# qpc001/Feature_Base_Pointcloud_Registration

Measured on AMD Instinct MI355X. Metric: registered scans/sec + pose RMSE vs ref, 64×1800 synthetic Velodyne, higher is better.
Workload: dtype f32; 1 GPU; C2: 64x1800 HDL-64-style scans, ~100k-pt local corner+surf map; 1024 independent scan-to-map jobs per GPU per step (C4-style independent jobs); parallelism=single GPU, imu_deskew=False, exact_voxel_order=0

## Files before the change

feature_base_pointcloud_registration_amd/csrc/fbr_api.hip:

```cpp
#include <hip/hip_runtime.h>

#include <algorithm>
#include <atomic>
#include <chrono>
#include <condition_variable>
#include <cmath>
#include <cstdio>
#include <cstdlib>
#include <cstring>
#include <dlfcn.h>
#include <functional>
#include <map>
#include <mutex>
#include <set>
#include <string>
#include <thread>
#include <vector>

#include "fbr_common.h"
#include "fbr_imu.h"
#include "fbr_kernels.h"
#include "fbr_msg.h"

using namespace fbr;
// ... 443 lines not shown
  if (!sb.stream_mode && !pk && !c->staged_24) return FBR_ERR_STATE;
  int32_t* owner = c->d_owner + j0 * c->HW;
  OwnerTag ot;
  const int trc = next_owner_tag(c, &ot);
  if (trc) return trc;
  TIMED_ON(c, sb.st, "project", launch_project(sb.st, c->d_pts + i0 * c->NMAX, c->d_nin + i0, c->NMAX, sb.B, c->H,
                                               c->W, owner, c->d_err + j0, sb.stream_mode ? c->single_n : -1, pk, ot));
  TIMED_ON(c, sb.st, "extract",
           launch_extract(sb.st, c->d_pts + i0 * c->NMAX, c->NMAX, owner, sb.B, c->H, c->W, c->d_rowcnt + j0 * c->H,
                          c->d_choff + j0 * c->H * (c->W / 32 + 1),
                          c->d_cloud + j0 * c->HW, c->d_col + j0 * c->HW, c->d_range + j0 * c->HW,
                          c->d_start + j0 * c->H, c->d_end + j0 * c->H, c->d_nvalid + j0, desk, pk, ot));
  return FBR_OK;
}

bool packed_scans_enabled() {
  static const bool v = [] {
    const char* e = std::getenv("FBR_PACKED_SCANS");
    return e ? std::atoi(e) != 0 : true;
  }();
  return v;
}

bool feat_surf_window() {
  static const bool v = [] {
    const char* e = std::getenv("FBR_FEAT_SURF_WINDOW");
    return e ? std::atoi(e) != 0 : true;
  }();
  return v;
}

int stage_features(fbr_ctx* c, const Sub& sb, bool stream_mode, bool err_clear = false, bool labels_out = false) {
  const int64_t j0 = sb.j0, HW = c->HW, H = c->H;
  FeatArgs a{};
  a.B = sb.B;
  a.H = c->H;
  a.W = c->W;
  a.cloud = c->d_cloud + j0 * HW;
  a.col = c->d_col + j0 * HW;
  a.range = c->d_range + j0 * HW;
  a.start_ring = c->d_start + j0 * H;
  a.end_ring = c->d_end + j0 * H;
  a.nvalid = c->d_nvalid + j0;
  a.edge_thr = c->P.edge_threshold;
  a.surf_thr = c->P.surf_threshold;
  if (stream_mode) {
    a.stream = c->d_sstream;
    a.label = c->d_label_stream;
  } else {
    CK(hipMemsetAsync(c->d_sstate + j0, 0, sizeof(StreamState) * sb.B, sb.st));
    a.stream = c->d_sstate + j0;
    a.label = c->d_label + j0 * HW;
  }
  a.corner_slot = c->d_corner_slot + j0 * H * kCornerPerRing;
  a.corner_cnt = c->d_corner_cnt + j0 * H;
  a.err = c->d_err + j0;
  a.surf_full = labels_out || !feat_surf_window() ? 1 : 0;
  a.carry = stream_mode ? 1 : 0;
  a.fresh = stream_mode ? 0 : 1;
  feat_caps(c->W, a);
  a.gscratch = c->d_feat_scratch + j0 * H * a.gslot_bytes;
  a.stamps = c->d_feat_stamps ? c->d_feat_stamps + j0 * H * 12 : nullptr;
  if (!err_clear) CK(hipMemsetAsync(c->d_err + j0, 0, sizeof(int32_t) * sb.B, sb.st));
  TIMED_ON(c, sb.st, "features", launch_features(sb.st, a));
  if (!stream_mode && c->diag_err_job >= sb.in0 && c->diag_err_job < sb.in0 + sb.B)
    CK(hipMemsetD32Async((hipDeviceptr_t)(c->d_err + j0 + (c->diag_err_job - sb.in0)), 1, 1, sb.st));
  VgRing v{};
  v.cloud = a.cloud;
  v.label = a.label;
  v.start_ring = a.start_ring;
  v.end_ring = a.end_ring;
  v.B = sb.B;
  v.H = c->H;
  v.HW = HW;
  v.cap = c->W;
  v.leaf = c->P.odometry_surf_leaf_size;
  v.out = c->d_surf_ring + j0 * HW;
  v.stride_out = c->W;
  v.cnt_out = c->d_surf_ring_cnt + j0 * H;
  v.dbg = std::getenv("FBR_VR_DBG") ? std::atoi(std::getenv("FBR_VR_DBG")) : 0;
  v.exact = c->P.exact_voxel_order ? 1 : 0;
  v.stamps = a.stamps;
  v.kernel = c->diag_ring_filter;
  TIMED_ON(c, sb.st, "voxel_ring", launch_voxel_ring(sb.st, v));
  TIMED_ON(c, sb.st, "concat",
           launch_concat(sb.st, sb.B, c->H, c->W, a.corner_slot, a.corner_cnt, v.out, v.cnt_out,
                         c->d_corner_all + j0 * HW, HW, c->d_ncorner + j0, c->d_surf_all + j0 * HW, HW,
                         c->d_nsurf + j0, c->d_ring_box + j0 * H * kRingBox));
  c->ring_box_valid = true;
  return FBR_OK;
}

GnArgs gn_args(fbr_ctx* c, const Sub& sb, bool trace) {
  const int64_t j0 = sb.j0, HW = c->HW, ib = j0 * c->items_per_job;
  const int mi = std::max(1, c->P.max_iterations);
  GnArgs a{};
#ifdef FBR_KNN_STATS
  a.knn_stats = knn_stats_buffer();
#endif
  a.B = sb.B;
  a.max_iter = c->P.max_iterations;
  a.cornerDS = c->d_cornerDS + j0 * HW;
  a.capc = HW;
  a.ncds = c->d_ncds + j0;
  a.surfDS = c->d_surfDS + j0 * HW;
  a.caps = HW;
  a.nsds = c->d_nsds + j0;
  a.mc = c->grid_c.view();
  a.ms = c->grid_s.view();
  a.gn = c->d_gn + j0;
  a.guess = c->d_guess + (int64_t)sb.in0 * 6;
  a.items = c->d_items + ib;
  a.nitems = c->d_nitems + sb.k;
  a.item_range = c->d_item_range + j0 * 2;
  a.partial = c->d_partial + ib * 32;
  a.max_items = sb.B * c->items_per_job;
  a.edge_min = c->P.edge_feature_min_valid_num;
  a.surf_min = c->P.surf_feature_min_valid_num;
  for (int k = 0; k < 3; ++k) a.crop_half[k] = c->P.crop_half[k];
  a.rot_tol = c->P.rotation_tollerance;
  a.z_tol = c->P.z_tollerance;
  a.pose_out = c->d_pose_out + j0 * 6;
  a.stats = c->d_stats + j0;
  a.trace = trace ? c->d_trace + j0 * c->P.max_iterations * 6 : nullptr;
  a.nbr = c->d_nbr + ib * 5 * 256;
  a.fitc = c->d_fitc + ib * 6 * 256;
  a.fits = c->d_fits + ib * 256;
  a.nsame = c->d_nsame + ib * 256;
  static const int fit_cache = [] {
    const char* e = std::getenv("FBR_FIT_CACHE");
    return e ? std::atoi(e) : 1;
  }();
  a.fit_cache = fit_cache;
  a.iter_flags = c->d_iter_flags + (int64_t)sb.k * mi;
  a.items_flag = c->d_iter_flags + (int64_t)kMaxSub * mi + sb.k;
  a.iter_cnt = c->d_iter_cnt + (int64_t)sb.k * 4 * mi;
  if (c->d_bin) {
    const int64_t slots = (int64_t)c->max_items * 256;
    a.fb_list = c->d_fb_list + ib * 256;
    a.bin_list = c->d_fb_list + slots + ib * 256;
    a.qblk = c->d_fb_list + 2 * slots + ib * 256;
    a.bin = c->d_bin + (int64_t)sb.k * 3 * c->bin_nb;
    a.nb_c = (int)c->bin_nb_c;
    a.nb_s = (int)(c->bin_nb - c->bin_nb_c);
  }
  a.desk_mode = c->desk_any ? c->d_desk_mode + sb.in0 : nullptr;
  a.desk = c->desk_any ? c->d_desk + sb.in0 : nullptr;
  a.nocrop = c->map_nocrop ? 1 : 0;
  a.deg_carry = sb.stream_mode ? c->stream_degenerate : 0;
  if (c->direct_gen && sb.stream_mode && sb.B == 1 && c->d_direct) {
    a.direct = c->d_direct;
    a.direct_done = c->d_direct_done;
    a.direct_gen = c->direct_gen;
    a.nvalid = c->d_nvalid + j0;
    a.ncorner = c->d_ncorner + j0;
    a.nsurf = c->d_nsurf + j0;
    a.ferr = c->d_err + j0;
    a.cropcnt = c->d_cropcnt + (int64_t)sb.in0 * 2;
  }
  return a;
}

int batch_quiesce(fbr_ctx* c);
int drop_staged_batch(fbr_ctx* c) {
  const int rc = batch_quiesce(c);
  c->staged_B = 0;
// ... 1799 lines not shown
}

}

int fbr_process_batch(fbr_ctx* c, const fbr_point_xyzirt* const* scans, const int64_t* n_in, int n_jobs,
                      float* poses_inout, fbr_reg_stats* stats) {
  if (!c || !scans || !n_in || !poses_inout || n_jobs < 0) return FBR_ERR_INVALID_ARG;
  for (int j = 0; j < n_jobs; ++j) {
    if (n_in[j] < 0 || n_in[j] > c->NMAX) return FBR_ERR_CAPACITY;
    if (n_in[j] && !scans[j]) return FBR_ERR_INVALID_ARG;
  }
  if (n_jobs == 0) return FBR_OK;
  if (!c->has_map) return FBR_ERR_NO_MAP;
  CK(enter(c));
  int rc = ingest_init(c);
  if (rc) return rc;
  c->ing.h2d_bytes = 0.0;
  const int nb = (n_jobs + c->Bcap - 1) / c->Bcap;
  auto first = [&](int b) { return b * c->Bcap; };
  auto count = [&](int b) { return std::min(c->Bcap, n_jobs - b * c->Bcap); };
  rc = ingest_upload(c, 0, scans, n_in, count(0));
  for (int b = 0; b < nb && !rc; ++b) {
    const int slot = b & 1, j0 = first(b), B = count(b);
    int up_rc = FBR_OK;
    std::thread up;
    if (b + 1 < nb)
      up = std::thread([&, b] { up_rc = ingest_upload(c, slot ^ 1, scans + first(b + 1), n_in + first(b + 1), count(b + 1)); });
    rc = ingest_stage(c, slot, n_in + j0, B, poses_inout + 6 * j0);
    if (!rc) rc = fbr_batch_launch(c);
    if (!rc) rc = fbr_batch_wait(c);
    if (!rc) rc = fbr_batch_results(c, poses_inout + 6 * j0, stats ? stats + j0 : nullptr);
    if (up.joinable()) up.join();
    if (!rc) rc = up_rc;
  }
  (void)fbr_sync(c->ing.cstream);
  if (c->ing.xstream) (void)fbr_sync(c->ing.xstream);
  c->d_pts = c->ing.d_pts_slot[0];
  if (rc) (void)drop_staged_batch(c);
  return rc;
}

int fbr_debug_counters(long long* launches, long long* host_syncs, long long* flag_polls, int reset) {
  DebugCounters& d = debug_counters();
  if (launches) *launches = d.launches.load();
  if (host_syncs) *host_syncs = d.host_syncs.load();
  if (flag_polls) *flag_polls = d.flag_polls.load();
  if (reset) {
    d.launches = 0;
    d.host_syncs = 0;
    d.flag_polls = 0;
  }
  return FBR_OK;
}

extern "C" int fbr_diag_host_times(long long* out4, int reset) {
  DebugCounters& d = debug_counters();
  for (int k = 0; k < 4; ++k) {
    if (out4) out4[k] = d.host_ns[k].load();
    if (reset) d.host_ns[k] = 0;
  }
  return FBR_OK;
}

extern "C" int fbr_diag_wait_stats(long long* out4, int reset) {
  DebugCounters& d = debug_counters();
  std::atomic<long long>* v[4] = {&d.flag_fallbacks, &d.waits_over_1ms, &d.wait_max_ns, &d.stream_queries};
  for (int k = 0; k < 4; ++k) {
    if (out4) out4[k] = v[k]->load();
    if (reset) *v[k] = 0;
  }
  return FBR_OK;
}

extern "C" int fbr_diag_batch_times(long long* out2, int reset) {
  DebugCounters& d = debug_counters();
  for (int k = 0; k < 2; ++k) {
    if (out2) out2[k] = d.batch_ns[k].load();
    if (reset) d.batch_ns[k] = 0;
  }
  return FBR_OK;
}

extern "C" int fbr_diag_ring_filter(fbr_ctx* c, int kernel) {
  if (!c || (kernel != -1 && kernel != 0 && kernel != 2)) return FBR_ERR_INVALID_ARG;
  c->diag_ring_filter = kernel;
  return FBR_OK;
}

extern "C" int fbr_diag_force_capacity_error(fbr_ctx* c, int job) {
  if (!c) return FBR_ERR_INVALID_ARG;
  c->diag_err_job = job < 0 ? -1 : job;
  return FBR_OK;
}

int fbr_ingest_bytes(fbr_ctx* c, double* h2d_bytes) {
  if (!c || !h2d_bytes) return FBR_ERR_INVALID_ARG;
  *h2d_bytes = c->ing.h2d_bytes;
  return FBR_OK;
}

int fbr_voxel_grid(fbr_ctx* c, const fbr_point_xyzi* in, int64_t n, float leaf, fbr_point_xyzi* out, int64_t* n_out) {
  if (!c || n < 0 || (n && !in) || !(leaf > 0)) return FBR_ERR_INVALID_ARG;
  CK(enter(c));
  std::vector<fbr_point_xyzi> o;
  int rc = voxel_grid_once(c, in, n, leaf, o);
  if (rc) return rc;
  if (out) std::memcpy(out, o.data(), sizeof(fbr_point_xyzi) * o.size());
  if (n_out) *n_out = (int64_t)o.size();
  return FBR_OK;
}

extern "C" int fbr_diag_feature_stamps(fbr_ctx* c, unsigned long long* out ) {
  if (!c) return FBR_ERR_INVALID_ARG;
  CK(enter(c));
  const size_t n = (size_t)c->Bwork * c->H * 12;
  if (!c->d_feat_stamps) {
    CK(hipMalloc(&c->d_feat_stamps, sizeof(unsigned long long) * n));
    CK(hipMemset(c->d_feat_stamps, 0, sizeof(unsigned long long) * n));
    return FBR_OK;
  }
  if (out) CK(fbr_memcpy_sync(out, c->d_feat_stamps, sizeof(unsigned long long) * n, hipMemcpyDeviceToHost));
  return FBR_OK;
}

int fbr_set_profiling(fbr_ctx* c, int enable) {
  if (!c) return FBR_ERR_INVALID_ARG;
  c->profiling = enable != 0;
  return FBR_OK;
}

int fbr_set_profiling_kernels(fbr_ctx* c, const char* names) {
  if (!c) return FBR_ERR_INVALID_ARG;
  c->profile_only.clear();
  if (!names) return FBR_OK;
  std::string cur;
  for (const char* q = names;; ++q) {
    if (*q == ',' || *q == '\0') {
      if (!cur.empty()) c->profile_only.insert(cur);
      cur.clear();
      if (*q == '\0') break;
    } else {
      cur.push_back(*q);
    }
  }
  return FBR_OK;
}

int fbr_kernel_time(fbr_ctx* c, const char* kernel, double* total_ms, int64_t* launches) {
  if (!c || !kernel) return FBR_ERR_INVALID_ARG;
  CK(enter(c));
  auto itr = c->timers.find(kernel);
  if (itr == c->timers.end()) {
    if (total_ms) *total_ms = 0.0;
    if (launches) *launches = 0;
    return FBR_OK;
  }
  KernelTimer& t = itr->second;
  for (auto& pr : t.pending) {
    CK(hipEventSynchronize(pr.second));
    float ms = 0.0f;
    CK(hipEventElapsedTime(&ms, pr.first, pr.second));
    t.total_ms += ms;
    t.launches += 1;
    t.pool.push_back(pr);
  }
  t.pending.clear();
  if (total_ms) *total_ms = t.total_ms;
// ... 203 lines not shown
```

feature_base_pointcloud_registration_amd/csrc/fbr_kernels.h:

```cpp
#pragma once
#include <hip/hip_ext.h>
#include <hip/hip_runtime.h>
#include <stdint.h>

#include <algorithm>
#include <atomic>

#include "fbr_common.h"

namespace fbr {

struct LaunchTimer {
  hipEvent_t start = nullptr, stop = nullptr;
  int launched = 0;
};
inline LaunchTimer& launch_timer() {
  static thread_local LaunchTimer t;
  return t;
}

struct DebugCounters {
  std::atomic<long long> launches{0}, host_syncs{0}, flag_polls{0};
  std::atomic<long long> host_ns[4] = {0, 0, 0, 0};
  std::atomic<long long> batch_ns[2] = {0, 0};
// ... 68 lines not shown
  int surf_full = 1;
  int carry = 0;
  int fresh = 0;
};
size_t features_lds_bytes(const FeatArgs& a, int nwv);
size_t features_gslot_bytes(const FeatArgs& a);
void launch_features(hipStream_t s, const FeatArgs& a);

struct VgSet {
  const float4* in;
  int64_t stride_in;
  const int32_t* cnt_in;
  int64_t cap;
  float4* out;
  int64_t stride_out;
  int32_t* cnt_out;
  uint32_t* scratch;
  float leaf;
  int nseg;
  int morton;
  int exact;
  const float* box;
  int box_n;
  int64_t box_stride;
};
constexpr int64_t kVgScratch = 5;
struct VgArgs {
  VgSet s[2];
  int32_t* err = nullptr;
};
constexpr int32_t kVgErrLookback = 16;
constexpr int64_t kVgLdsCap = 4096;
void launch_voxel_grid(hipStream_t s, const VgArgs& a);

struct DevArena {
  char* base = nullptr;
  size_t cap = 0, used = 0;
};
inline size_t arena_bytes(size_t b) { return (std::max<size_t>(b, 1) + 255) & ~(size_t)255; }
inline hipError_t arena_reserve(DevArena& a, size_t bytes, hipStream_t s) {
  a.used = 0;
  if (bytes <= a.cap) return hipSuccess;
  hipError_t e = hipStreamSynchronize(s);
  if (e != hipSuccess) return e;
  if (a.base) (void)hipFree(a.base);
  a.base = nullptr;
  a.cap = 0;
  const size_t nc = std::max(bytes + bytes / 4, (size_t)1 << 20);
  e = hipMalloc((void**)&a.base, nc);
  if (e == hipSuccess) a.cap = nc;
  return e;
}
template <typename T>
T* arena_take(DevArena& a, size_t bytes) {
  const size_t b = arena_bytes(bytes);
  if (!a.base || a.used + b > a.cap) return nullptr;
  T* p = reinterpret_cast<T*>(a.base + a.used);
  a.used += b;
  return p;
}
inline void arena_free(DevArena& a) {
  if (a.base) (void)hipFree(a.base);
  a = DevArena{};
}

constexpr int64_t kVgLargeMin = 32768;
int voxel_grid_large(hipStream_t s, DevArena& ar, const float4* in, int64_t n, float leaf, int morton, int exact,
                     float4* out, int32_t* d_nout);

struct VgRing {
  const float4* cloud;
  const int8_t* label;
  const int32_t* start_ring;
  const int32_t* end_ring;
  int B, H;
  int64_t HW;
  int64_t cap;
  float leaf;
  float4* out;
  int64_t stride_out;
  int32_t* cnt_out;
  int dbg;
  int kernel = -1;
  int exact;
  unsigned long long* stamps;
};
void launch_voxel_ring(hipStream_t s, const VgRing& a);

constexpr int kRingBox = 12;
void launch_concat(hipStream_t s, int B, int H, int W, const float4* corner_slot, const int32_t* corner_cnt,
                   const float4* surf_ring, const int32_t* surf_ring_cnt, float4* corner_all, int64_t capc,
                   int32_t* n_corner, float4* surf_all, int64_t caps, int32_t* n_surf, float* ring_box);

struct MapGrid {
  const float4* pts;
  const int32_t* cell_start;
  GridDesc g;
  const float4* by_id;
  const unsigned long long* hkeys;
  const int32_t* hvals;
};

struct DevGrid {
  float4* pts = nullptr;
  int32_t* cs = nullptr;
  unsigned long long* hkeys = nullptr;
  int32_t* hvals = nullptr;
  GridDesc g{};
  MapGrid view() const { return MapGrid{pts, cs, g, pts + g.n_points, hkeys, hvals}; }
};
constexpr int64_t kDenseGridCells = (int64_t)1 << 26;
void free_grid(DevGrid& d);
int grid_build_device(hipStream_t s, DevArena& ar, const float4* pts, int64_t n, float invx, float inv,
                      bool force_sparse, DevGrid& out);

struct JobResult;
struct GnArgs {
  int B, max_iter;
  int one_item;
  int rest_grid;
  int one_part;
  const float4* cornerDS;
  int64_t capc;
  const int32_t* ncds;
  const float4* surfDS;
  int64_t caps;
  const int32_t* nsds;
  MapGrid mc, ms;
  GnState* gn;
  const float* guess;
  int4* items;
  int32_t* nitems;
  int32_t* item_range;
  double* partial;
  int max_items;
  int edge_min, surf_min;
  float crop_half[3];
  float rot_tol, z_tol;
  float* pose_out;
  fbr_reg_stats* stats;
  float* trace;
  int32_t* nbr;
  float* fitc;
  int8_t* fits;
  int8_t* nsame;
  int fit_cache;
  unsigned long long* iter_flags;
  unsigned long long* items_flag;
  int32_t* iter_cnt;
  int32_t* fb_list;
  int32_t* bin_list;
  int32_t* qblk;
  int32_t* bin;
  int nb_c, nb_s;
  const int32_t* desk_mode;
  const fbr_deskew_table* desk;
  int nocrop;
  int deg_carry;
  unsigned long long* knn_stats;
  JobResult* direct;
  int32_t* direct_done;
  int32_t direct_gen;
  const int32_t* nvalid;
  const int32_t* ncorner;
  const int32_t* nsurf;
  const int32_t* ferr;
// ... 36 lines not shown
```

feature_base_pointcloud_registration_amd/csrc/k_voxel.hip:

```cpp
#include <rocprim/device/device_radix_sort.hpp>
#include <rocprim/device/device_scan.hpp>

#include "fbr_common.h"
#include "fbr_introsort.h"
#include "fbr_kernels.h"

#include <algorithm>
#include <atomic>
#include <mutex>
#include <cstdlib>
#include <type_traits>

namespace fbr {


__device__ __forceinline__ uint32_t spread3_10(uint32_t v) {
  v &= 0x3FFu;
  v = (v | (v << 16)) & 0x030000FFu;
  v = (v | (v << 8)) & 0x0300F00Fu;
  v = (v | (v << 4)) & 0x030C30C3u;
  v = (v | (v << 2)) & 0x09249249u;
  return v;
}

// ... 985 lines not shown

__device__ __forceinline__ uint64_t shfl_xor_u64(uint64_t x, int m) {
  const uint32_t lo = __shfl_xor((uint32_t)x, m), hi = __shfl_xor((uint32_t)(x >> 32), m);
  return ((uint64_t)hi << 32) | lo;
}

template <int E>
__device__ __forceinline__ void wave_bitonic_u64(uint64_t (&v)[E], int lane) {
  constexpr int N = 64 * E;
#pragma unroll
  for (int k = 2; k <= N; k <<= 1) {
#pragma unroll
    for (int j = k >> 1; j > 0; j >>= 1) {
      if (j >= E) {
        const int m = j / E;
        const bool lower = (lane & m) == 0;
        const bool asc = ((lane * E) & k) == 0;
        const bool take_min = lower == asc;
#pragma unroll
        for (int e = 0; e < E; ++e) {
          const uint64_t o = shfl_xor_u64(v[e], m);
          v[e] = take_min ? key_min(o, v[e]) : key_max(o, v[e]);
        }
      } else {
#pragma unroll
        for (int e = 0; e < E; ++e) {
          if (e & j) continue;
          const bool asc = ((lane * E + e) & k) == 0;
          const uint64_t a = v[e], b = v[e | j];
          const uint64_t lo = key_min(a, b), hi = key_max(a, b);
          v[e] = asc ? lo : hi;
          v[e | j] = asc ? hi : lo;
        }
      }
    }
  }
}

__device__ __forceinline__ void wave_lds_sync() {
  __builtin_amdgcn_fence(__ATOMIC_SEQ_CST, "workgroup");
  __builtin_amdgcn_wave_barrier();
}

template <int E>
__device__ int vr_sort_runs(const uint32_t* kb, int R, uint16_t* sid, uint16_t* vst, int lane) {
  uint64_t v[E];
#pragma unroll
  for (int e = 0; e < E; ++e) {
    const int g = lane * E + e;
    v[e] = g < R ? (((uint64_t)kb[g] << 16) | (uint64_t)g) : kF64KeyMax;
  }
  wave_bitonic_u64<E>(v, lane);
  const uint32_t lo = __shfl_up((uint32_t)v[E - 1], 1), hi = __shfl_up((uint32_t)(v[E - 1] >> 32), 1);
  const uint64_t prev_last = ((uint64_t)hi << 32) | lo;
  bool hd[E];
  int nh = 0;
#pragma unroll
  for (int e = 0; e < E; ++e) {
    const int g = lane * E + e;
    const uint64_t pk = e ? (v[e - 1] >> 16) : (prev_last >> 16);
    hd[e] = g < R && (g == 0 || (v[e] >> 16) != pk);
    nh += hd[e] ? 1 : 0;
  }
  int inc = nh;
#pragma unroll
  for (int o = 1; o < 64; o <<= 1) {
    const int y = __shfl_up(inc, o);
    if (lane >= o) inc += y;
  }
  const int V = __shfl(inc, 63);
  int vi = inc - nh;
  wave_lds_sync();
#pragma unroll
  for (int e = 0; e < E; ++e) {
    const int g = lane * E + e;
    if (g < R) sid[g] = (uint16_t)(v[e] & 0xFFFFull);
    if (hd[e]) vst[vi++] = (uint16_t)g;
  }
  if (lane == 0) vst[V] = (uint16_t)R;
  wave_lds_sync();
  return V;
}

template <int KQ>
__global__ void __launch_bounds__(256) __attribute__((amdgpu_waves_per_eu(KQ <= 8 ? 8 : 1, KQ <= 8 ? 8 : 10)))
k_voxel_ring_q(VgRing A) {
  constexpr int NW = 4;
  extern __shared__ __attribute__((aligned(16))) unsigned char smem[];
  __shared__ float mmx[NW][6];
  __shared__ int cntw[NW], runw[NW];
  const int tid = threadIdx.x, lane = tid & 63, w = tid >> 6;
  const int slot = blockIdx.x, job = slot / A.H;
  const int s = A.start_ring[slot], e = A.end_ring[slot];
  float4* out = A.out + (int64_t)slot * A.stride_out;
  if (e <= s) {
    if (tid == 0) A.cnt_out[slot] = 0;
    return;
  }
  int sp6[6], ep6[6];
  bool all6 = true;
#pragma unroll
  for (int j = 0; j < 6; ++j) {
    sp6[j] = (s * (6 - j) + e * j) / 6;
    ep6[j] = (s * (5 - j) + e * (j + 1)) / 6 - 1;
    all6 = all6 && sp6[j] < ep6[j];
  }
  auto in_seg = [&](int k) {
    if (all6) return k <= ep6[5];
    bool in = false;
#pragma unroll
    for (int j = 0; j < 6; ++j) in |= sp6[j] < ep6[j] && k >= sp6[j] && k <= ep6[j];
    return in;
  };
  const float4* CL = A.cloud + (int64_t)job * A.HW + s;
  const int8_t* LB = A.label + (int64_t)job * A.HW + s;
  const int len = min(e - s, (int)A.cap);
  const uint64_t lt = (1ull << lane) - 1ull;
  const int qlen = (((len + NW - 1) / NW) + 63) & ~63;
  const int q0 = min(len, w * qlen), q1 = min(len, q0 + qlen);
  float4 pt[KQ];
  bool cd[KQ];
  int lb[KQ];
#pragma unroll
  for (int u = 0; u < KQ; ++u) {
    const int ic = min(q0 + 64 * u + lane, len - 1);
    lb[u] = LB[ic];
    pt[u] = CL[ic];
  }
#pragma unroll
  for (int u = 0; u < KQ; ++u) asm volatile("" ::"v"(lb[u]), "v"(pt[u].x), "v"(pt[u].y), "v"(pt[u].z));
#pragma unroll
  for (int u = 0; u < KQ; ++u) cd[u] = q0 + 64 * u + lane < q1 && lb[u] <= 0;
  float mn[3] = {FLT_MAX, FLT_MAX, FLT_MAX}, mx[3] = {-FLT_MAX, -FLT_MAX, -FLT_MAX};
  int nw = 0;
#pragma unroll
  for (int u = 0; u < KQ; ++u) {
    cd[u] = cd[u] && in_seg(s + q0 + 64 * u + lane);
    if (cd[u]) {
      const float v[3] = {pt[u].x, pt[u].y, pt[u].z};
#pragma unroll
      for (int d = 0; d < 3; ++d) {
        mn[d] = (v[d] < mn[d]) ? v[d] : mn[d];
        mx[d] = (mx[d] < v[d]) ? v[d] : mx[d];
      }
    }
    nw += __popcll(__ballot(cd[u]));
  }
#pragma unroll
  for (int d = 0; d < 3; ++d)
    for (int o = 32; o > 0; o >>= 1) {
      const float a = __shfl_xor(mn[d], o), b = __shfl_xor(mx[d], o);
      mn[d] = (a < mn[d]) ? a : mn[d];
      mx[d] = (mx[d] < b) ? b : mx[d];
    }
  if (lane == 0) {
    for (int d = 0; d < 3; ++d) {
      mmx[w][d] = mn[d];
      mmx[w][3 + d] = mx[d];
    }
    cntw[w] = nw;
  }
  __syncthreads();
  int n = 0, base = 0;
#pragma unroll
  for (int ww = 0; ww < NW; ++ww) {
    base += ww < w ? cntw[ww] : 0;
    n += cntw[ww];
  }
  if (n == 0) {
    if (tid == 0) A.cnt_out[slot] = 0;
    return;
  }
#pragma unroll
  for (int d = 0; d < 3; ++d) {
    mn[d] = mmx[0][d];
    mx[d] = mmx[0][3 + d];
#pragma unroll
    for (int ww = 1; ww < NW; ++ww) {
      mn[d] = (mmx[ww][d] < mn[d]) ? mmx[ww][d] : mn[d];
      mx[d] = (mx[d] < mmx[ww][3 + d]) ? mmx[ww][3 + d] : mx[d];
    }
  }
  VgGrid G;
  G.init(mn, mx, A.leaf, false);
  const int cap = (int)A.cap;
  uint32_t* kb = (uint32_t*)smem;
  uint16_t* off = (uint16_t*)(kb + cap + 1);
  uint16_t* rst = off + cap;
#pragma unroll
  for (int u = 0; u < KQ; ++u) {
    const uint64_t b = __ballot(cd[u]);
    const int pos = base + __popcll(b & lt);
    if (cd[u]) {
      if (G.overflow) {
        out[pos] = CL[q0 + 64 * u + lane];
      } else {
        kb[pos] = G.key(pt[u]);
        off[pos] = (uint16_t)(q0 + 64 * u + lane);
      }
    }
    base += __popcll(b);
  }
  if (G.overflow) {
    if (tid == 0) A.cnt_out[slot] = n;
    return;
  }
  __syncthreads();
  const int tq = (((n + NW - 1) / NW) + 63) & ~63;
  const int t0w = min(n, w * tq), t1w = min(n, t0w + tq);
  constexpr int KR = KQ;
  uint32_t rk[KR];
  uint64_t hb[KR];
  int nr = 0;
#pragma unroll
  for (int u = 0; u < KR; ++u) {
    const int t = t0w + 64 * u + lane;
    const bool valid = t < t1w;
    const uint32_t key = valid ? kb[t] : 0u;
    const uint32_t prev = (valid && t > 0) ? kb[t - 1] : 0u;
    rk[u] = key;
    hb[u] = __ballot(valid && (t == 0 || key != prev));
    nr += __popcll(hb[u]);
  }
  if (lane == 0) runw[w] = nr;
  __syncthreads();
  int R = 0, rq = 0;
#pragma unroll
  for (int ww = 0; ww < NW; ++ww) {
    rq += ww < w ? runw[ww] : 0;
    R += runw[ww];
  }
#pragma unroll
  for (int u = 0; u < KR; ++u) {
    if ((hb[u] >> lane) & 1ull) {
      const int r = rq + __popcll(hb[u] & lt);
      kb[r] = rk[u];
      rst[r] = (uint16_t)(t0w + 64 * u + lane);
    }
    rq += __popcll(hb[u]);
  }
  if (tid == 0) rst[R] = (uint16_t)n;
  __syncthreads();
  uint16_t* sid = (uint16_t*)kb;
  uint16_t* vst = sid + cap + 1;
  __shared__ int vcount;
  if (R <= 512) {
    if (w == 0) {
      const int V = R <= 256 ? vr_sort_runs<4>(kb, R, sid, vst, lane) : vr_sort_runs<8>(kb, R, sid, vst, lane);
      if (lane == 0) vcount = V;
    }
  } else {
    uint64_t* scr = reinterpret_cast<uint64_t*>(out);
    for (int r = tid; r < R; r += 256) {
      const uint32_t key = kb[r];
      int rank = 0;
      for (int j = 0; j < R; ++j) {
        const uint32_t kj = kb[j];
        rank += (kj < key || (kj == key && j < r)) ? 1 : 0;
      }
      scr[rank] = ((uint64_t)key << 16) | (uint64_t)r;
    }
    __syncthreads();
    if (w == 0) {
      int V = 0;
      for (int g0 = 0; g0 < R; g0 += 64) {
        const int g = g0 + lane;
        const uint64_t x = g < R ? scr[g] : ~0ull;
        const uint64_t px = (g > 0 && g < R) ? scr[g - 1] : ~0ull;
        const bool hd = g < R && (g == 0 || (x >> 16) != (px >> 16));
        const uint64_t b = __ballot(hd);
        wave_lds_sync();
        if (g < R) sid[g] = (uint16_t)(x & 0xFFFFull);
        if (hd) vst[V + __popcll(b & lt)] = (uint16_t)g;
        V += __popcll(b);
      }
      if (lane == 0) {
        vst[V] = (uint16_t)R;
        vcount = V;
      }
    }
  }
  __syncthreads();
  const int V = vcount;
  for (int vv = tid; vv < V; vv += 256) {
    const int g0 = vst[vv], g1 = vst[vv + 1];
    float4 c = make_float4(0.f, 0.f, 0.f, 0.f);
    int cnt = 0;
    for (int g = g0; g < g1; ++g) {
      const int rid = sid[g];
      const int ta = rst[rid], tb = rst[rid + 1];
      for (int t = ta; t < tb; t += 8) {
        float4 pp[8];
#pragma unroll
        for (int u = 0; u < 8; ++u) pp[u] = CL[off[min(t + u, tb - 1)]];
#pragma unroll
        for (int u = 0; u < 8; ++u)
          if (t + u < tb) {
            if (cnt == 0) {
              c = pp[u];
            } else {
              c.x += pp[u].x;
              c.y += pp[u].y;
              c.z += pp[u].z;
              c.w += pp[u].w;
            }
            ++cnt;
          }
      }
    }
    const float fc = (float)cnt;
    out[vv] = make_float4(c.x / fc, c.y / fc, c.z / fc, c.w / fc);
  }
  if (tid == 0) A.cnt_out[slot] = V;
}

bool vr_four_waves(int nseg) { return nseg > 256; }

size_t voxel_ring_lds_bytes(const VgRing& a, int threads, int kpt) {
  const int nw = threads / 64;
  size_t b = sizeof(uint32_t) * ((size_t)(nw + 1) * 256 + nw) + sizeof(float) * nw * 6 + sizeof(int) * kpt * nw;
  b = (b + 15) & ~(size_t)15;
  return b + (size_t)a.cap * 2 * (sizeof(uint32_t) + sizeof(uint16_t)) + (size_t)(2 * a.cap + 1) * sizeof(uint16_t) + 16;
}

void launch_voxel_ring(hipStream_t s, const VgRing& a) {
  const int nseg = a.B * a.H;
  if (nseg <= 0) return;
  const int kpt = (int)((a.cap + 511) / 512);
  auto go = [&](auto ex) {
    constexpr bool E = decltype(ex)::value;
    if (kpt <= 2)
      fbr_launch((k_voxel_ring<512, 2, E>), dim3(nseg), dim3(512), voxel_ring_lds_bytes(a, 512, 2), s, a);
    else if (kpt <= 4)
      fbr_launch((k_voxel_ring<512, 4, E>), dim3(nseg), dim3(512), voxel_ring_lds_bytes(a, 512, 4), s, a);
    else
      fbr_launch((k_voxel_ring<512, 8, E>), dim3(nseg), dim3(512), voxel_ring_lds_bytes(a, 512, 8), s, a);
  };
  if (a.exact) {
    go(std::true_type{});
  } else if ((a.kernel < 0 ? vr_four_waves(nseg) : a.kernel == 2) && a.dbg == 0 && a.cap <= 4096) {
    const size_t lds = (((size_t)a.cap + 1) * 4 + (size_t)a.cap * 2 + ((size_t)a.cap + 1) * 2 + 15) & ~(size_t)15;
    if (a.cap <= 4 * 64 * 8) fbr_launch(k_voxel_ring_q<8>, dim3(nseg), dim3(256), lds, s, a);
    else fbr_launch(k_voxel_ring_q<16>, dim3(nseg), dim3(256), lds, s, a);
  } else {
    go(std::false_type{});
  }
}

bool vg_inplace() {
  static const bool v = [] {
    const char* e = std::getenv("FBR_VG_INPLACE");
    return e ? std::atoi(e) != 0 : true;
  }();
  return v;
}

size_t voxel_lds_bytes(const VgArgs& a, int threads, bool lds_mode) {
  const int nw = threads / 64;
  size_t b = sizeof(uint32_t) * ((size_t)(nw + 1) * 512 + nw) + sizeof(float) * nw * 6 + sizeof(int) * 4;
  b = (b + 15) & ~(size_t)15;
  if (lds_mode) {
    int64_t cap = 0;
    for (int k = 0; k < 2; ++k)
      if (a.s[k].nseg > 0) cap = std::max<int64_t>(cap, a.s[k].cap);
    b += (size_t)cap * 2 * (sizeof(uint32_t) + sizeof(uint16_t)) + 16;
  }
  return b;
}

constexpr int kVgIpKpl = 18;
constexpr int kVgSplitSlots = 16;
constexpr int kVgSplitRing = 1024;
constexpr int kVgSplitMaxDevices = 64;
int vg_split() {
  static const int v = [] {
    const char* e = std::getenv("FBR_VG_SPLIT");
    const int p = e ? std::atoi(e) : 8;
    return p < 2 ? 1 : std::min(p, 8);
  }();
  return v;
}

void launch_voxel_grid(hipStream_t s, const VgArgs& a) {
  const int nseg = a.s[0].nseg + a.s[1].nseg;
  if (nseg <= 0) return;
  int64_t cap = 0;
  for (int k = 0; k < 2; ++k)
    if (a.s[k].nseg > 0) cap = std::max<int64_t>(cap, a.s[k].cap);
  const bool exact = a.s[0].exact || a.s[1].exact;
  const int P = vg_split();
  if (!exact && P > 1 && cap > kVgLdsCap && vg_inplace() && nseg * P <= kVgSplitSlots) {
    static std::mutex mu;
    static unsigned long long* dev_flags[kVgSplitMaxDevices] = {};
    static bool dev_failed[kVgSplitMaxDevices] = {};
    int dev = -1;
    unsigned long long* flags = nullptr;
    if (hipGetDevice(&dev) == hipSuccess && dev >= 0 && dev < kVgSplitMaxDevices) {
      std::lock_guard<std::mutex> lk(mu);
      if (!dev_flags[dev] && !dev_failed[dev]) {
        unsigned long long* f = nullptr;
        const size_t bytes = sizeof(unsigned long long) * kVgSplitSlots * kVgSplitRing;
        if (hipMalloc(&f, bytes) == hipSuccess && hipMemset(f, 0, bytes) == hipSuccess) dev_flags[dev] = f;
        else dev_failed[dev] = true;
      }
      flags = dev_flags[dev];
    }
    static std::atomic<unsigned> gen{0};
    if (flags) {
      const unsigned g = gen.fetch_add(1) + 1;
      const size_t lds = voxel_lds_bytes(a, 1024, false) + (size_t)1024 * kVgIpKpl * (sizeof(uint32_t) + sizeof(uint16_t));
      fbr_launch((k_voxel_grid_split<1024, kVgIpKpl>), dim3(nseg * P), dim3(1024), lds, s, a, P,
                 flags + (size_t)(g % kVgSplitRing) * kVgSplitSlots, g);
      return;
    }
  }
  auto go = [&](auto ex) {
    constexpr bool E = decltype(ex)::value;
    if (cap <= kVgLdsCap) {
      fbr_launch((k_voxel_grid<256, uint16_t, true, E>), dim3(nseg), dim3(256), voxel_lds_bytes(a, 256, true), s, a);
    } else if (vg_inplace()) {
      const size_t lds =
          voxel_lds_bytes(a, 1024, false) + (size_t)1024 * kVgIpKpl * (sizeof(uint32_t) + sizeof(uint16_t));
      fbr_launch((k_voxel_grid_ip<1024, kVgIpKpl, E>), dim3(nseg), dim3(1024), lds, s, a);
    } else {
      fbr_launch((k_voxel_grid<1024, uint32_t, false, E>), dim3(nseg), dim3(1024), voxel_lds_bytes(a, 1024, false),
                 s, a);
// ... 344 lines not shown
```

Before: 138,900 scans/s.

## Accumulate per-voxel run sums in LDS during key emission to skip gather

In the quad-wave ring voxel filter, each wave now segments consecutive equal-key points while it emits keys and accumulates running centroid sums into an LDS pool. In the final averaging pass, voxels made of a single sorted run that lies inside one wave's range read the precomputed sum instead of re-gathering points from global memory through the offset table. A w0 flag skips the intensity channel when it is not needed. This costs extra LDS (a staging area and a pool), extra wave syncs and ballots during emission, and falls back to the gather path when the pool overflows or a run spans waves.

```diff
diff --git a/feature_base_pointcloud_registration_amd/csrc/fbr_api.hip b/feature_base_pointcloud_registration_amd/csrc/fbr_api.hip
--- a/feature_base_pointcloud_registration_amd/csrc/fbr_api.hip
+++ b/feature_base_pointcloud_registration_amd/csrc/fbr_api.hip
@@ -549,6 +549,7 @@
   v.exact = c->P.exact_voxel_order ? 1 : 0;
   v.stamps = a.stamps;
   v.kernel = c->diag_ring_filter;
+  v.w0 = (!stream_mode && c->staged_pk && !(c->desk_any && !c->no_time_call)) ? 1 : 0;
   TIMED_ON(c, sb.st, "voxel_ring", launch_voxel_ring(sb.st, v));
   TIMED_ON(c, sb.st, "concat",
            launch_concat(sb.st, sb.B, c->H, c->W, a.corner_slot, a.corner_cnt, v.out, v.cnt_out,
@@ -2514,7 +2515,7 @@
 }
 
 extern "C" int fbr_diag_ring_filter(fbr_ctx* c, int kernel) {
-  if (!c || (kernel != -1 && kernel != 0 && kernel != 2)) return FBR_ERR_INVALID_ARG;
+  if (!c || kernel < -1 || kernel > 3) return FBR_ERR_INVALID_ARG;
   c->diag_ring_filter = kernel;
   return FBR_OK;
 }
diff --git a/feature_base_pointcloud_registration_amd/csrc/fbr_kernels.h b/feature_base_pointcloud_registration_amd/csrc/fbr_kernels.h
--- a/feature_base_pointcloud_registration_amd/csrc/fbr_kernels.h
+++ b/feature_base_pointcloud_registration_amd/csrc/fbr_kernels.h
@@ -174,6 +174,7 @@
   int32_t* cnt_out;
   int dbg;
   int kernel = -1;
+  int w0;
   int exact;
   unsigned long long* stamps;
 };
diff --git a/feature_base_pointcloud_registration_amd/csrc/k_voxel.hip b/feature_base_pointcloud_registration_amd/csrc/k_voxel.hip
--- a/feature_base_pointcloud_registration_amd/csrc/k_voxel.hip
+++ b/feature_base_pointcloud_registration_amd/csrc/k_voxel.hip
@@ -1091,13 +1091,30 @@
   return V;
 }
 
-template <int KQ>
+constexpr int kVrqGather = 0, kVrqSums0 = 1, kVrqSumsW = 2;
+
+struct VrqLds {
+  int o_x, o_pool, o_off, total;
+};
+__host__ __device__ inline VrqLds vrq_lds(int cap, int P, bool sums) {
+  VrqLds l;
+  l.o_x = ((cap + 1) * 4 + 15) & ~15;
+  int xb = (cap + 1) * 2;
+  if (sums && xb < 4 * 64 * 16) xb = 4 * 64 * 16;
+  l.o_pool = l.o_x + ((xb + 15) & ~15);
+  l.o_off = l.o_pool + (sums ? 4 * P * 16 : 0);
+  l.total = (l.o_off + cap * 2 + 15) & ~15;
+  return l;
+}
+template <int KQ, int kMode>
 __global__ void __launch_bounds__(256) __attribute__((amdgpu_waves_per_eu(KQ <= 8 ? 8 : 1, KQ <= 8 ? 8 : 10)))
-k_voxel_ring_q(VgRing A) {
+k_voxel_ring_q(VgRing A, int P) {
   constexpr int NW = 4;
+  constexpr bool kSums = kMode != kVrqGather;
+  constexpr int kRunDepth = KQ <= 8 ? 4 : 2;
   extern __shared__ __attribute__((aligned(16))) unsigned char smem[];
   __shared__ float mmx[NW][6];
-  __shared__ int cntw[NW], runw[NW];
+  __shared__ int cntw[NW], runw[NW], segw[NW], contw[NW];
   const int tid = threadIdx.x, lane = tid & 63, w = tid >> 6;
   const int slot = blockIdx.x, job = slot / A.H;
   const int s = A.start_ring[slot], e = A.end_ring[slot];
@@ -1137,7 +1154,10 @@
     pt[u] = CL[ic];
   }
 #pragma unroll
-  for (int u = 0; u < KQ; ++u) asm volatile("" ::"v"(lb[u]), "v"(pt[u].x), "v"(pt[u].y), "v"(pt[u].z));
+  for (int u = 0; u < KQ; ++u) {
+    if constexpr (kMode == kVrqSumsW) asm volatile("" ::"v"(lb[u]), "v"(pt[u].x), "v"(pt[u].y), "v"(pt[u].z), "v"(pt[u].w));
+    else asm volatile("" ::"v"(lb[u]), "v"(pt[u].x), "v"(pt[u].y), "v"(pt[u].z));
+  }
 #pragma unroll
   for (int u = 0; u < KQ; ++u) cd[u] = q0 + 64 * u + lane < q1 && lb[u] <= 0;
   float mn[3] = {FLT_MAX, FLT_MAX, FLT_MAX}, mx[3] = {-FLT_MAX, -FLT_MAX, -FLT_MAX};
@@ -1193,19 +1213,73 @@
   VgGrid G;
   G.init(mn, mx, A.leaf, false);
   const int cap = (int)A.cap;
+  const VrqLds L = vrq_lds(cap, P, kSums);
   uint32_t* kb = (uint32_t*)smem;
-  uint16_t* off = (uint16_t*)(kb + cap + 1);
-  uint16_t* rst = off + cap;
+  uint16_t* rst = (uint16_t*)(smem + L.o_x);
+  float4* stg = (float4*)(smem + L.o_x) + 64 * w;
+  float4* pool = (float4*)(smem + L.o_pool) + P * w;
+  uint16_t* off = (uint16_t*)(smem + L.o_off);
+  const int cbw = base;
+  float4 cs = make_float4(0.f, 0.f, 0.f, 0.f);
+  uint32_t ckey = 0u;
+  bool open = false;
+  int nseg = 0;
 #pragma unroll
   for (int u = 0; u < KQ; ++u) {
     const uint64_t b = __ballot(cd[u]);
-    const int pos = base + __popcll(b & lt);
+    const int j = __popcll(b & lt);
+    const int pos = base + j;
     if (cd[u]) {
       if (G.overflow) {
         out[pos] = CL[q0 + 64 * u + lane];
       } else {
         kb[pos] = G.key(pt[u]);
         off[pos] = (uint16_t)(q0 + 64 * u + lane);
+        if constexpr (kSums) stg[j] = make_float4(pt[u].x, pt[u].y, pt[u].z, kMode == kVrqSumsW ? pt[u].w : 0.0f);
+      }
+    }
+    if constexpr (kSums) {
+      const int m = __popcll(b);
+      if (m > 0 && !G.overflow) {
+        wave_lds_sync();
+        const uint32_t kj = lane < m ? kb[base + lane] : 0u;
+        const uint32_t kp = __shfl_up(kj, 1);
+        const bool hd = lane < m && (lane == 0 ? (!open || kj != ckey) : kj != kp);
+        const uint64_t hm = __ballot(hd);
+        const uint64_t lm = hm | 1ull;
+        const bool lead = (lm >> lane) & 1ull;
+        const uint64_t above = (lm >> lane) >> 1;
+        const int end = above ? lane + 1 + (int)__builtin_ctzll(above) : m;
+        if (lane == 0 && open && hd && nseg - 1 < P) pool[nseg - 1] = cs;
+        float4 c = cs;
+        int i = 0;
+        if (hd) {
+          c = stg[lane];
+          i = lane + 1;
+        }
+        if (lead) {
+          for (; i < end; i += kRunDepth) {
+            float4 p[kRunDepth];
+#pragma unroll
+            for (int q = 0; q < kRunDepth; ++q) p[q] = stg[min(i + q, end - 1)];
+#pragma unroll
+            for (int q = 0; q < kRunDepth; ++q)
+              if (i + q < end) {
+                c.x += p[q].x;
+                c.y += p[q].y;
+                c.z += p[q].z;
+                c.w += p[q].w;
+              }
+          }
+          const int sx = hd ? nseg + __popcll(hm & lt) : nseg - 1;
+          if (end < m && sx < P) pool[sx] = c;
+        }
+        const int ll = 63 - (int)__builtin_clzll(lm);
+        cs = make_float4(__shfl(c.x, ll), __shfl(c.y, ll), __shfl(c.z, ll), __shfl(c.w, ll));
+        ckey = __shfl(kj, m - 1);
+        open = true;
+        nseg += __popcll(hm);
+        wave_lds_sync();
       }
     }
     base += __popcll(b);
@@ -1214,7 +1288,14 @@
     if (tid == 0) A.cnt_out[slot] = n;
     return;
   }
-  __syncthreads();
+  if constexpr (kSums)
+    if (lane == 0 && open && nseg - 1 < P) pool[nseg - 1] = cs;
+  __syncthreads();
+  if constexpr (kSums)
+    if (lane == 0) {
+      segw[w] = nseg;
+      contw[w] = (nseg > 0 && cbw > 0 && kb[cbw] == kb[cbw - 1]) ? 1 : 0;
+    }
   const int tq = (((n + NW - 1) / NW) + 63) & ~63;
   const int t0w = min(n, w * tq), t1w = min(n, t0w + tq);
   constexpr int KR = KQ;
@@ -1252,6 +1333,7 @@
   __syncthreads();
   uint16_t* sid = (uint16_t*)kb;
   uint16_t* vst = sid + cap + 1;
+  static_assert(sizeof(uint32_t) == 2 * sizeof(uint16_t), "sid + vst fill kb's bytes");
   __shared__ int vcount;
   if (R <= 512) {
     if (w == 0) {
@@ -1291,8 +1373,42 @@
   }
   __syncthreads();
   const int V = vcount;
+  int cb[NW + 1], rb[NW], ct[NW];
+  if constexpr (kSums) {
+    cb[0] = 0;
+    int r = 0;
+#pragma unroll
+    for (int ww = 0; ww < NW; ++ww) {
+      cb[ww + 1] = cb[ww] + cntw[ww];
+      ct[ww] = contw[ww];
+      rb[ww] = r;
+      r += segw[ww] - ct[ww];
+    }
+  }
   for (int vv = tid; vv < V; vv += 256) {
     const int g0 = vst[vv], g1 = vst[vv + 1];
+    if constexpr (kSums) {
+      if (g1 - g0 == 1) {
+        const int rid = sid[g0];
+        const int ta = rst[rid], tb = rst[rid + 1];
+        int cbe = cb[1], rbw = rb[0], ctw = ct[0], ww = 0;
+#pragma unroll
+        for (int k = 1; k < NW; ++k)
+          if (ta >= cb[k]) {
+            cbe = cb[k + 1];
+            rbw = rb[k];
+            ctw = ct[k];
+            ww = k;
+          }
+        const int lr = rid - rbw + ctw;
+        if (tb <= cbe && lr < P) {
+          const float4 c = ((const float4*)(smem + L.o_pool))[P * ww + lr];
+          const float fc = (float)(tb - ta);
+          out[vv] = make_float4(c.x / fc, c.y / fc, c.z / fc, c.w / fc);
+          continue;
+        }
+      }
+    }
     float4 c = make_float4(0.f, 0.f, 0.f, 0.f);
     int cnt = 0;
     for (int g = g0; g < g1; ++g) {
@@ -1330,6 +1446,12 @@
   size_t b = sizeof(uint32_t) * ((size_t)(nw + 1) * 256 + nw) + sizeof(float) * nw * 6 + sizeof(int) * kpt * nw;
   b = (b + 15) & ~(size_t)15;
   return b + (size_t)a.cap * 2 * (sizeof(uint32_t) + sizeof(uint16_t)) + (size_t)(2 * a.cap + 1) * sizeof(uint16_t) + 16;
+}
+
+int vrq_pool(const VgRing& a) {
+  if (a.cap > 4 * 64 * 8) return 96;
+  const int room = 160 * 1024 / 8 - 256 - vrq_lds((int)a.cap, 0, true).total;
+  return std::max(16, std::min(128, room / (4 * 16) / 8 * 8));
 }
 
 void launch_voxel_ring(hipStream_t s, const VgRing& a) {
@@ -1347,10 +1469,18 @@
   };
   if (a.exact) {
     go(std::true_type{});
-  } else if ((a.kernel < 0 ? vr_four_waves(nseg) : a.kernel == 2) && a.dbg == 0 && a.cap <= 4096) {
-    const size_t lds = (((size_t)a.cap + 1) * 4 + (size_t)a.cap * 2 + ((size_t)a.cap + 1) * 2 + 15) & ~(size_t)15;
-    if (a.cap <= 4 * 64 * 8) fbr_launch(k_voxel_ring_q<8>, dim3(nseg), dim3(256), lds, s, a);
-    else fbr_launch(k_voxel_ring_q<16>, dim3(nseg), dim3(256), lds, s, a);
+  } else if ((a.kernel < 0 ? vr_four_waves(nseg) : a.kernel >= 2) && a.dbg == 0 && a.cap <= 4096) {
+    const int P = vrq_pool(a);
+    const int mode = a.kernel == 3 ? kVrqGather : a.w0 ? kVrqSums0 : kVrqSumsW;
+    const size_t lds = (size_t)vrq_lds((int)a.cap, P, mode != kVrqGather).total;
+    auto gq = [&](auto kq) {
+      constexpr int KQ = decltype(kq)::value;
+      if (mode == kVrqGather) fbr_launch((k_voxel_ring_q<KQ, kVrqGather>), dim3(nseg), dim3(256), lds, s, a, P);
+      else if (mode == kVrqSums0) fbr_launch((k_voxel_ring_q<KQ, kVrqSums0>), dim3(nseg), dim3(256), lds, s, a, P);
+      else fbr_launch((k_voxel_ring_q<KQ, kVrqSumsW>), dim3(nseg), dim3(256), lds, s, a, P);
+    };
+    if (a.cap <= 4 * 64 * 8) gq(std::integral_constant<int, 8>{});
+    else gq(std::integral_constant<int, 16>{});
   } else {
     go(std::false_type{});
   }
```

New measurement: 128,200 scans/s. 0.923x the previous value.
